# nipponjo/tts-arabic-pytorch

Measured on AMD Instinct MI355X. Metric: audio samples/sec (FastPitch+HiFi-GAN, synthetic 64-phoneme inputs), higher is better.
Workload: dtype f32

## Files before the change

tts-arabic-pytorch_amd/csrc/conv_wino4.hip:

```cpp
#include <cstdlib>
#include <cstring>

#include <algorithm>
#include <vector>

#include "conv_mfma_common.hpp"
#include "bfo.hpp"

namespace ttsamd {

typedef float w4_f32x4 __attribute__((ext_vector_type(4)));
typedef float w4_f32x2 __attribute__((ext_vector_type(2)));

template <int K, int NOCT_, int NSTAGE_, int EPI_ = 0, int PT_ = 6, int LP_ = 1>
struct Wino4Geo {
    static constexpr bool PT7 = PT_ == 7;
    static_assert(PT_ == 6 || (PT7 && (K == 7 || K == 11)), "seven-point groups: k = 7 / 11");
    static constexpr int WM = 2, WN = 2;
    static constexpr int NSF = K == 1 ? 0 : (K == 3 ? 1 : (K == 7 ? 2 : (PT7 ? 3 : 4)));
    static constexpr int NL = (!PT7 && (K == 7 || K == 1)) ? 1 : 0;
    static constexpr int GSF = PT7 ? 7 : 6;
    static constexpr int SSF = PT7 ? 4 : 3;
    static constexpr int NG = PT7 ? (K == 7 ? 13 : 20) : (K == 1 ? 4 : (K == 3 ? 6 : (K == 7 ? 16 : 23)));
    static constexpr int NGQ = PT7 ? NG : ((NG + 1) & ~1);
    static constexpr bool WSHARE = K == 1;
    static constexpr int NGW = WSHARE ? 1 : NGQ;
    static constexpr int NPL = PT7 ? (EPI_ == 3 ? 9 : 7) : ((NL || EPI_ == 3) ? 8 : 6);
    static constexpr int NPOS = K == 1 ? 4 : (K == 3 ? 6 : (K == 7 ? 10 : 14));
    static constexpr int NOCT = NOCT_, NSTAGE = NSTAGE_;
    static constexpr int NPH = PT7 ? ((K == 11 && LP_ == 2) ? 2 : 1) : (K == 11 ? 2 : 1);
    static constexpr int PH0 = PT7 ? 8 : 12;
    static constexpr int NGPM = NPH == 1 ? NG : 12;
    static_assert(NPH == 1 || (PH0 <= NGPM && NG - PH0 <= NGPM), "phase sizes");
    static constexpr int CO_BLK = WM * 32;
    static constexpr int NTUP = WN * 32;
    static constexpr int NT_BLK = 4 * NTUP;
    static constexpr int BUF4 = NOCT * 2 * NGPM * NTUP;
    static constexpr int PF = 4;
    static constexpr int NM = 4;
    __host__ __device__ static constexpr int glo(int ph) { return NPH == 1 ? 0 : PH0 * ph; }
    __host__ __device__ static constexpr int ngp(int ph) { return NPH == 1 ? NG : (ph == 0 ? PH0 : NG - PH0); }
    __host__ __device__ static constexpr int ngq(int ph) { return NPH == 1 ? NGQ : (PT7 ? ngp(ph) : 12); }
    __host__ __device__ static constexpr int gfirst(int g) {
        return g < GSF * NSF ? SSF * (g / GSF) : 3 * NSF + (g - 6 * NSF);
    }
    __host__ __device__ static constexpr int glast(int g) {
        if (PT7) return 4 * (g / 7) + (g % 7 == 6 ? 6 : 5);
        return g < 6 * NSF ? (3 * (g / 6) + 5 < NPOS ? 3 * (g / 6) + 5 : NPOS - 1) : 3 * NSF + (g - 6 * NSF);
    }
    __host__ __device__ static constexpr int plane(int g) {
        if (PT7) return g % 7;
        return g < 6 * NSF ? g % 6 : ((g - 6 * NSF) == 0 ? 0 : ((g - 6 * NSF) == 1 ? 6 : ((g - 6 * NSF) == 2 ? 7 : 5)));
    }
    __host__ __device__ static constexpr int rplane(int j) { return PT7 ? (j == 0 ? 0 : (j == 1 ? 7 : (j == 2 ? 8 : 6))) : (j == 0 ? 0 : (j == 1 ? 6 : (j == 2 ? 7 : 5))); }
    __host__ __device__ static constexpr int mlo(int ph) { return gfirst(glo(ph)); }
    __host__ __device__ static constexpr int mhi(int ph) {
        int m = 0;
        for (int g = glo(ph); g < glo(ph) + ngp(ph); ++g) m = glast(g) > m ? glast(g) : m;
        return m;
    }
    static_assert(mhi(NPH - 1) == NPOS - 1 && mlo(0) == 0, "the groups cover the window and nothing past it");
    __host__ __device__ static constexpr int npos(int ph) { return mhi(ph) - mlo(ph) + 1; }
    static constexpr int NPOSP = npos(0) > npos(NPH - 1) ? npos(0) : npos(NPH - 1);
    __host__ __device__ static constexpr int ngap(int ph) { return NOCT * ngp(ph) * NM; }
    __host__ __device__ static constexpr int sph(int ph) { return ((ph - (NSTAGE - 1)) % NPH + NPH) % NPH; }
    __host__ __device__ static constexpr int sgap(int ph) { return ngap(sph(ph)); }
    static constexpr int JSF = 10;
    __host__ __device__ static constexpr int sflo(int ph) { return glo(ph) / 7; }
    __host__ __device__ static constexpr bool inph(int ph, int g) { return g >= glo(ph) && g < glo(ph) + ngp(ph); }
    __host__ __device__ static constexpr int glast_ph(int ph) { return glo(ph) + ngp(ph) - 1; }
    __host__ __device__ static constexpr int nwj(int ph) {
        return PT7 ? JSF * (glast_ph(ph) / 7 - sflo(ph)) + (glast_ph(ph) % 7 == 0 ? 3 : JSF) : NOCT * ngp(ph);
    }
    static_assert(!PT7 || (NOCT == 1 && glo(0) % 7 <= 1 && glo(NPH - 1) % 7 <= 1 &&
                           (glast_ph(0) % 7 == 0 || glast_ph(0) % 7 >= 5) && glast_ph(NPH - 1) % 7 >= 5),
                  "seven-point phases: start on V0 / V1 of a sub-filter (the partial sums are formed per phase), end on V0 or the last row");
    __host__ __device__ static constexpr int fdiv4(int e) { return e >= 0 ? e / 4 : -((3 - e) / 4); }
    __host__ __device__ static constexpr int vlo(int ph) { return fdiv4(mlo(ph) - (K - 1) / 2); }
    __host__ __device__ static constexpr int nvec(int ph) { return fdiv4(mhi(ph) - (K - 1) / 2) - vlo(ph) + 1; }
    static constexpr int NVP = nvec(0) > nvec(NPH - 1) ? nvec(0) : nvec(NPH - 1);
    __host__ __device__ static constexpr int nljv(int ph) { return NOCT * 2 * nvec(ph); }
    static constexpr int DAV = (K == 3 || K == 1) ? 8 : 16;
    __host__ __device__ static constexpr int tw0v(int ph) { return DAV + 2 * nljv(ph); }
    __host__ __device__ static constexpr int wsv(int ph) { return (sgap(ph) - tw0v(ph)) / nwj(ph); }
    static_assert(LP_ != 1 || (wsv(0) >= 1 && wsv(NPH - 1) >= 1), "one write job per gap at most (vector loads)");
    static constexpr int RAWW = 320;
    static constexpr int NROW = 2 * NOCT;
    static constexpr int RAW_BYTES = 4 * (NROW * RAWW * 4 + 16);
    static constexpr int DAT = K == 7 ? 16 : (K == 11 ? 12 : 8);
    __host__ __device__ static constexpr int nrj(int ph) { return NROW * ((npos(ph) + 1) / 2); }
    __host__ __device__ static constexpr bool loads_in(int ph) { return ph == 0; }
    __host__ __device__ static constexpr int tr_r0(int ph) { return loads_in(ph) ? DAT + 2 * NROW : 0; }
    __host__ __device__ static constexpr int tw0t(int ph) { return tr_r0(ph) + nrj(ph) + 1; }
    __host__ __device__ static constexpr int wst(int ph) { return (sgap(ph) - tw0t(ph)) / nwj(ph); }
    static_assert(LP_ != 2 || (wst(0) >= 1 && wst(NPH - 1) >= 1), "one write job per gap at most (strip path)");
    static constexpr int QX = WSHARE ? 0 : (NOCT * ngq(0)) % PF;
    static constexpr int QMAIN = NOCT * ngq(0) - QX;
    static_assert(QX == 0 || (NPH == 1 && NOCT == 1 && QMAIN >= 2 * PF), "extra queue slots: one phase, one octet");
    static_assert((WSHARE ? NOCT : NOCT * ngq(NPH - 1)) % PF == 0 || QX != 0, "queue slots line up across steps");
    static_assert((size_t)NSTAGE * BUF4 * 16 + (LP_ == 2 ? RAW_BYTES : 0) <= 80 * 1024, "two blocks per CU");
    static_assert(NPH == 1 || NOCT == 1, "phases split an octet's groups");
};

__device__ __host__ constexpr int wino4_tile(int d, int ntup) { return (4 * ntup / (4 * d)) * (4 * d); }

template <int K, int NOCT_, int NSTAGE_, int EPI, int LP, int PT = 6>
__global__ __launch_bounds__(256, kConvMinWaves) void conv1d_wino4_f32(const ConvParams p) {
    extern __shared__ __attribute__((aligned(16))) float4 smem4[];
    using G = Wino4Geo<K, NOCT_, NSTAGE_, EPI, PT, LP>;
    constexpr bool PT7 = G::PT7;
    constexpr int WN = G::WN, NSF = G::NSF, NOCT = G::NOCT, NSTAGE = G::NSTAGE, NPL = G::NPL, NGPM = G::NGPM;
    constexpr int CO_BLK = G::CO_BLK, NTUP = G::NTUP, NT_BLK = G::NT_BLK, PF = G::PF;
    constexpr int NPH = G::NPH, NPOSP = G::NPOSP, NM = G::NM;
    constexpr bool D1 = LP == 1, TR = LP == 2;
    static_assert(D1 || TR, "window path");
    const int dil = D1 ? 1 : p.dil;
    const int nt_eff = wino4_tile(dil, NTUP), ntup_eff = nt_eff / 4;
    const int tiles_y = p.CoutP / CO_BLK;
    const int per_tile = tiles_y * p.ksplit;
    const unsigned sidx = blockIdx.x, xcd = sidx & 7u, u = sidx >> 3;
    const int yk = (int)(u % (unsigned)per_tile);
    const unsigned gt = (u / (unsigned)per_tile) * 8u + xcd;
    const int n_tiles_x = (p.Nout + nt_eff - 1) / nt_eff;
    int b = (int)(gt / (unsigned)n_tiles_x);
    int q0 = (int)(gt % (unsigned)n_tiles_x) * nt_eff;
    if (p.compact) {
        int tile = 0;
        if (!live_tile(p.lens_out, p.len_out_mul, p.Nout, nt_eff, p.batch, gt, b, tile)) return;
        b = __builtin_amdgcn_readfirstlane(b);
        q0 = __builtin_amdgcn_readfirstlane(tile) * nt_eff;
    } else if (b >= p.batch) {
        return;
    }
    const int tid = threadIdx.x, lane = tid & 63, wid = tid >> 6;
    const int wm = wid / WN, wn = wid % WN;
    const int ks = yk / tiles_y;
    const int co_blk0 = (yk - ks * tiles_y) * CO_BLK;
    int n_out = p.Nout;
    if (p.lens_out) n_out = min(n_out, (int)p.lens_out[b] * p.len_out_mul);
    if (q0 >= n_out) return;
    int in_len = p.Lin;
    if (p.lens_in) in_len = min(in_len, (int)p.lens_in[b] * p.len_in_mul);

    const int x_cs = p.x_cs, CoutP = p.CoutP;
    const int chunks_all = p.Cin / (8 * NOCT);
    const int c_beg = (int)((int64_t)ks * chunks_all / p.ksplit), n_chunks = (int)((int64_t)(ks + 1) * chunks_all / p.ksplit);
    const int n_groups = (p.Cin / 8) * G::NGW;
    const float* __restrict__ xb = p.x + (int64_t)b * p.x_bs;
    const float in_slope = p.in_slope;

    float ep_bias = 0.f;
    if (tid < CO_BLK && p.bias) ep_bias = p.bias[min(co_blk0 + tid, p.Cout - 1)];

    const int kk = lane >> 5, l31 = lane & 31;
    const int pe = wn * 32 + l31;
    const int col_e = dil == 1 ? 4 * pe : (pe / dil) * 4 * dil + pe % dil;
    f32x16 acc[NPL];
#pragma unroll
    for (int g = 0; g < NPL; ++g)
#pragma unroll
        for (int r = 0; r < 16; ++r) acc[g][r] = 0.f;
    constexpr bool preload = EPI == 3;
    if constexpr (preload) {
        const int wm_s = __builtin_amdgcn_readfirstlane(wm);
        const int row0 = co_blk0 + wm_s * 32;
        const int qv = q0 + col_e;
        const int voff = (qv < n_out ? qv : 0) * 4;
        {
            const int r_cs = p.r_cs;
            const bfo_i4 rs = bfo_rsrc(p.res + (int64_t)b * p.r_bs, (unsigned)p.Cout * (unsigned)r_cs * 4u);
            const int vk = 4 * kk * r_cs * 4;
#pragma unroll
            for (int r = 0; r < 16; ++r) {
                const w4_f32x4 t = __builtin_bit_cast(w4_f32x4, bfo_ld16(rs, voff + vk, (row0 + (r & 3) + 8 * (r >> 2)) * r_cs * 4, 0));
                acc[G::rplane(0)][r] = t.x; acc[G::rplane(1)][r] = t.y; acc[G::rplane(2)][r] = t.z; acc[G::rplane(3)][r] = t.w;
            }
        }
        if (p.mode != 0) {
            const int y_cs_ = p.y_cs;
            const bfo_i4 ys = bfo_rsrc(p.y + (int64_t)b * p.y_bs, (unsigned)p.Cout * (unsigned)y_cs_ * 4u);
            const int vk = 4 * kk * y_cs_ * 4;
#pragma unroll
            for (int r = 0; r < 16; ++r) {
                const w4_f32x4 t = __builtin_bit_cast(w4_f32x4, bfo_ld16(ys, voff + vk, (row0 + (r & 3) + 8 * (r >> 2)) * y_cs_ * 4, 0));
                acc[G::rplane(0)][r] += t.x; acc[G::rplane(1)][r] += t.y; acc[G::rplane(2)][r] += t.z; acc[G::rplane(3)][r] += t.w;
            }
        }
    }

    const bfo_i4 wrs = bfo_rsrc(K == 1 ? p.w : (PT7 ? p.w_wino44 : p.w_wino4), (unsigned)n_groups * 2u * (unsigned)CoutP * 16u);
    const int wv = (kk * CoutP + co_blk0 + wm * 32 + l31) * 16;
    const int wstep = 2 * CoutP * 16, wlast = (n_groups - 1) * wstep;
    int wso = c_beg * NOCT * G::NGW * wstep;
    w4_f32x4 aq[PF + G::QX];
    if constexpr (G::QX == 0) {
#pragma unroll
        for (int g = 0; g < PF; ++g) {
            aq[g] = __builtin_bit_cast(w4_f32x4, bfo_ld16(wrs, wv, wso, 0));
            wso = min(wso + wstep, wlast);
        }
    } else {
#pragma unroll
        for (int g = 0; g < PF + G::QX; ++g)
            aq[g] = __builtin_bit_cast(w4_f32x4, bfo_ld16(wrs, wv, min(wso + (g < PF ? g : G::QMAIN + g - PF) * wstep, wlast), 0));
    }

    const int sh = __builtin_amdgcn_readfirstlane((tid >> 7) & 1), skk = __builtin_amdgcn_readfirstlane((tid >> 6) & 1);
    w4_f32x2 sx[D1 ? 1 : NOCT][D1 ? 1 : NPOSP];
    w4_f32x4 sv[D1 ? NOCT : 1][2][D1 ? G::NVP : 1];
    w4_f32x2 ta[NOCT], tb[NOCT];
    w4_f32x2 tf[PT7 ? 5 : 1], te[PT7 ? 4 : 1], td[PT7 ? 3 : 1], th[PT7 ? 2 : 1];
    const int spe = min(lane, ntup_eff - 1);
    const int xw0 = (q0 + 4 * lane) * 4;
    constexpr int pad_c = (K - 1) / 2;
    const int ch_off = (4 * sh + skk) * x_cs;

#define TTS_VJOB_IDX(PH, J)                                                                          \
        const int nv_ = G::nvec(PH);                                                                 \
        const int ol_ = (J) / (2 * nv_), pp_ = ((J) / nv_) % 2, vi_ = (J) % nv_;
#define TTS_VLOAD_JOB(PH, J, XSO)                                                                    \
    {                                                                                                \
        TTS_VJOB_IDX(PH, J)                                                                          \
        const bfo_i4 xrs_ = bfo_rsrc(xb + ((XSO) + ch_off + (8 * ol_ + 2 * pp_) * x_cs), (unsigned)in_len * 4u);     \
        sv[ol_][pp_][vi_] = __builtin_bit_cast(w4_f32x4, bfo_ld16(xrs_, xw0 + 16 * (G::vlo(PH) + vi_), 0, 0));      \
    }
#define TTS_VACT_JOB(PH, A)                                                                          \
    {                                                                                                \
        TTS_VJOB_IDX(PH, (A) / 2)                                                                    \
        if ((A) % 2 == 0) {                                                                          \
            sv[ol_][pp_][vi_].x = bfo_lrelu(sv[ol_][pp_][vi_].x, in_slope);                          \
            sv[ol_][pp_][vi_].y = bfo_lrelu(sv[ol_][pp_][vi_].y, in_slope);                          \
        } else {                                                                                     \
            sv[ol_][pp_][vi_].z = bfo_lrelu(sv[ol_][pp_][vi_].z, in_slope);                          \
            sv[ol_][pp_][vi_].w = bfo_lrelu(sv[ol_][pp_][vi_].w, in_slope);                          \
        }                                                                                            \
    }
    float* const strip = reinterpret_cast<float*>(smem4 + NSTAGE * G::BUF4) + wid * (G::NROW * G::RAWW + 4);
    const int tr_a = (q0 - pad_c * dil) & ~3;
    const int tr_off = q0 + (dil == 1 ? 4 * spe : (spe / dil) * 4 * dil + spe % dil) - pad_c * dil - tr_a;
    w4_f32x4 rv[TR ? G::NROW : 1][2];
// ... 74 lines not shown
            const int s3 = 3 * (g_ / 6), i_ = g_ % 6;                                                \
             \
            if (i_ == 0) v2 = 4.f * TTS_SX(s3) + (TTS_SX(s3 + 4) - 5.f * TTS_SX(s3 + 2));           \
            else if (i_ == 1) {                                                                      \
                ta[ol_] = TTS_SX(s3 + 4) - 4.f * TTS_SX(s3 + 2);                                     \
                tb[ol_] = TTS_SX(s3 + 3) - 4.f * TTS_SX(s3 + 1);                                     \
                v2 = ta[ol_] + tb[ol_];                                                              \
            } else if (i_ == 2) v2 = ta[ol_] - tb[ol_];                                              \
            else if (i_ == 3) {                                                                      \
                ta[ol_] = TTS_SX(s3 + 4) - TTS_SX(s3 + 2);                                           \
                tb[ol_] = 2.f * (TTS_SX(s3 + 3) - TTS_SX(s3 + 1));                                   \
                v2 = ta[ol_] + tb[ol_];                                                              \
            } else if (i_ == 4) v2 = ta[ol_] - tb[ol_];                                              \
            else v2 = 4.f * TTS_SX(s3 + 1) + (TTS_SX(s3 + 5 < G::NPOS ? s3 + 5 : s3) - 5.f * TTS_SX(s3 + 3));           \
        } else {                                                                                     \
            v2 = TTS_SX(3 * NSF + (g_ - 6 * NSF));                                                   \
        }                                                                                            \
        if constexpr (!PT7) (WR)[2 * ((ol_ * 2 * NGPM + gl_) * NTUP)] = v2;                          \
    }

    const float4* sB = smem4 + kk * NGPM * NTUP + wn * 32 + l31;
    w4_f32x2* sW = reinterpret_cast<w4_f32x2*>(smem4 + skk * NGPM * NTUP + lane) + sh;
    float4 bq[2];

    {
#pragma unroll
        for (int st = 0; st < NSTAGE - 1; ++st) {
            const int ph = st % NPH;
            const int xso = min(c_beg + st / NPH, n_chunks - 1) * 8 * NOCT * x_cs;
            if constexpr (D1) {
#pragma unroll
                for (int J = 0; J < G::nljv(ph); ++J) TTS_VLOAD_JOB(ph, J, xso)
#pragma unroll
                for (int J = 0; J < 2 * G::nljv(ph); ++J) TTS_VACT_JOB(ph, J)
            } else {
                if (G::loads_in(ph)) {
#pragma unroll
                    for (int J = 0; J < 2 * G::NROW; ++J) TTS_TLOAD_JOB(J, xso)
#pragma unroll
                    for (int J = 0; J < 2 * G::NROW; ++J) TTS_TSTORE_JOB(J)
                }
#pragma unroll
                for (int J = 0; J < G::nrj(ph); ++J) TTS_TREAD_JOB(ph, J)
            }
            w4_f32x2* wr = sW + 2 * st * G::BUF4;
#pragma unroll
            for (int J = 0; J < G::nwj(ph); ++J) TTS_WRITE_JOB(ph, J, wr)
        }
    }
    __syncthreads();
    bq[0] = sB[0];

    int stage = 0;
    for (int c = c_beg; c < n_chunks; ++c) {
#pragma unroll
        for (int ph = 0; ph < NPH; ++ph) {
            const int tph = (ph + NSTAGE - 1) % NPH;
            const int xso = min(c + (ph + NSTAGE - 1) / NPH, n_chunks - 1) * 8 * NOCT * x_cs;
            const int stage_next = (stage + 1 == NSTAGE) ? 0 : stage + 1;
            const int stage_fill = (stage == 0) ? NSTAGE - 1 : stage - 1;
            w4_f32x2* wr = sW + 2 * stage_fill * G::BUF4;
            const float4* rd = sB + stage * G::BUF4;
            const int sn = (c + 1 < n_chunks || ph + 1 < NPH) ? stage_next : stage;
#pragma unroll
            for (int gs = 0; gs < NOCT * G::ngq(ph); ++gs) {
                const int ol = gs / G::ngq(ph), gl = gs % G::ngq(ph);
                const int qs = G::WSHARE ? ol % PF : ((G::QX && gs >= G::QMAIN) ? PF + gs - G::QMAIN : gs % PF);
                const w4_f32x4 a4 = aq[qs];
                if constexpr (G::QX != 0) {
                    const int nx = gs < G::QMAIN - PF ? gs + PF : (gs < G::QMAIN ? G::NGQ + gs + PF - G::QMAIN : G::NGQ + gs);
                    aq[qs] = __builtin_bit_cast(w4_f32x4, bfo_ld16(wrs, wv, min(wso + nx * wstep, wlast), 0));
                    if (gs == G::NGQ - 1) wso += G::NGQ * wstep;
                } else if (!G::WSHARE || gl == G::ngq(ph) - 1) {
                    aq[qs] = __builtin_bit_cast(w4_f32x4, bfo_ld16(wrs, wv, wso, 0));
                    wso = min(wso + wstep, wlast);
                }
                if (gl >= G::ngp(ph)) continue;
                const int r = ol * G::ngp(ph) + gl;
                const int cur = r & 1, nxt = cur ^ 1;
                const int plane = G::plane(G::glo(ph) + gl);
                if (r + 1 < NOCT * G::ngp(ph)) bq[nxt] = rd[(((r + 1) / G::ngp(ph)) * 2 * NGPM + (r + 1) % G::ngp(ph)) * NTUP];
                else if (NSTAGE >= 3) bq[nxt] = sB[sn * G::BUF4];
                __builtin_amdgcn_sched_barrier(0);
                const float bv[4] = {bq[cur].x, bq[cur].y, bq[cur].z, bq[cur].w};
#pragma unroll
                for (int m = 0; m < NM; ++m) {
                    acc[plane] = __builtin_amdgcn_mfma_f32_32x32x2f32(a4[m], bv[m], acc[plane], 0, 0, 0);
                    const int t = r * NM + m;
                    if constexpr (D1) {
                        if (t < G::nljv(tph)) TTS_VLOAD_JOB(tph, t, xso)
                        if (t >= G::DAV && t - G::DAV < 2 * G::nljv(tph)) TTS_VACT_JOB(tph, t - G::DAV)
                        if (t >= G::tw0v(tph) && (t - G::tw0v(tph)) % G::wsv(tph) == 0 &&
                            (t - G::tw0v(tph)) / G::wsv(tph) < G::nwj(tph))
                            TTS_WRITE_JOB(tph, (t - G::tw0v(tph)) / G::wsv(tph), wr)
                    } else {
                        if (G::loads_in(tph) && t < 2 * G::NROW) TTS_TLOAD_JOB(t, xso)
                        if (G::loads_in(tph) && t >= G::DAT && t < G::DAT + 2 * G::NROW) TTS_TSTORE_JOB(t - G::DAT)
                        if (t >= G::tr_r0(tph) && t - G::tr_r0(tph) < G::nrj(tph)) TTS_TREAD_JOB(tph, t - G::tr_r0(tph))
                        if (t >= G::tw0t(tph) && (t - G::tw0t(tph)) % G::wst(tph) == 0 && (t - G::tw0t(tph)) / G::wst(tph) < G::nwj(tph))
                            TTS_WRITE_JOB(tph, (t - G::tw0t(tph)) / G::wst(tph), wr)
                    }
                    __builtin_amdgcn_sched_barrier(0);
                }
            }
            __syncthreads();
            if (NSTAGE < 3) bq[0] = sB[sn * G::BUF4];
            else if ((NOCT * G::ngp(ph)) % 2 != 0) bq[0] = bq[1];
            stage = stage_next;
        }
    }
#undef TTS_TLOAD_JOB
#undef TTS_TSTORE_JOB
#undef TTS_TREAD_JOB
#undef TTS_VLOAD_JOB
#undef TTS_VACT_JOB
#undef TTS_VJOB_IDX
#undef TTS_SXV
#undef TTS_SX
#undef TTS_WRITE_JOB

    constexpr int LDS_F = CO_BLK * NT_BLK + CO_BLK;
    constexpr int LPR = NT_BLK / 4;
    static_assert(LPR == 64, "one wave instruction per row");
    float* ep = reinterpret_cast<float*>(smem4);
    float* epb = ep + LDS_F - CO_BLK;
    float* __restrict__ yb = p.y + (int64_t)b * p.y_bs;
    const float* __restrict__ rb = (p.res && !preload) ? p.res + (int64_t)b * p.r_bs : nullptr;
    const int mode = p.mode, relu_out = p.relu_out, Cout = p.Cout;
    const float div = p.div;
    __syncthreads();
    if (tid < CO_BLK) epb[tid] = ep_bias;
#pragma unroll
    for (int r = 0; r < 16; ++r) {
        const int row = wm * 32 + (r & 3) + 8 * (r >> 2) + 4 * kk;
        const float s12 = acc[1][r] + acc[2][r], d12 = acc[1][r] - acc[2][r];
        const float s34 = acc[3][r] + acc[4][r], d34 = acc[3][r] - acc[4][r];
        float y0 = acc[0][r] + s12 + s34;
        float y1 = d12 + 2.f * d34;
        float y2 = s12 + 4.f * s34;
        float y3 = d12 + 8.f * d34 + acc[PT7 ? 6 : 5][r];
        if constexpr (NSF == 0) { y0 = acc[0][r]; y1 = 0.f; y2 = 0.f; y3 = acc[5][r]; }
        if constexpr (PT7) {
            y0 += acc[5][r];
            y1 += 0.5f * acc[5][r];
            y2 += 0.25f * acc[5][r];
            y3 += 0.125f * acc[5][r];
            if constexpr (NPL == 9) {
                y1 += acc[7][r];
                y2 += acc[8][r];
            }
        } else if constexpr (NPL == 8) {
            y1 += acc[6][r];
            y2 += acc[7][r];
        }
        if (pe < ntup_eff) {
            if (dil == 1) {
                *reinterpret_cast<float4*>(ep + row * NT_BLK + col_e) = make_float4(y0, y1, y2, y3);
            } else {
                ep[row * NT_BLK + col_e] = y0;
                ep[row * NT_BLK + col_e + dil] = y1;
                ep[row * NT_BLK + col_e + 2 * dil] = y2;
                ep[row * NT_BLK + col_e + 3 * dil] = y3;
            }
        }
    }
    __syncthreads();
    constexpr int NR = CO_BLK / 4;
    const int col = lane * 4, q = q0 + col;
    if (q >= n_out || col >= nt_eff) return;
    const bool full = q + 3 < n_out;
    if (p.ksplit > 1) {
        float* __restrict__ pb = p.splitk_ws + ((int64_t)ks * p.batch + b) * Cout * p.Nout;
#pragma unroll 4
        for (int it = 0; it < NR; ++it) {
            const int rl = wid + it * 4;
            const int co = co_blk0 + rl;
            if (co >= Cout) continue;
            const float4 a4 = *reinterpret_cast<const float4*>(ep + rl * NT_BLK + col);
            float* yp = pb + (int64_t)co * p.Nout + q;
            if (full && (p.Nout & 3) == 0) {
                *reinterpret_cast<float4*>(yp) = a4;
            } else {
                const float v[4] = {a4.x, a4.y, a4.z, a4.w};
#pragma unroll
                for (int e = 0; e < 4; ++e)
                    if (q + e < n_out) yp[e] = v[e];
            }
        }
        return;
    }
    const float* __restrict__ scale = K == 1 ? p.scale : nullptr;
    const bool plain_act = K != 1 || (relu_out < 2 && scale == nullptr);
    if (plain_act && (preload || (!rb && mode == 0))) {
        const float lo = relu_out == 1 ? 0.f : -__builtin_inff();
        const bool do_div = preload && mode == 2;
#pragma unroll 4
        for (int it = 0; it < NR; ++it) {
            const int rl = wid + it * 4;
            const int co = co_blk0 + rl;
            if (co >= Cout) continue;
            const float bsv = epb[rl];
            const float4 a4 = *reinterpret_cast<const float4*>(ep + rl * NT_BLK + col);
            float v[4] = {fmaxf(a4.x + bsv, lo), fmaxf(a4.y + bsv, lo), fmaxf(a4.z + bsv, lo), fmaxf(a4.w + bsv, lo)};
            if (do_div) {
#pragma unroll
                for (int e = 0; e < 4; ++e) v[e] = v[e] / div;
            }
            float* yp = yb + (int64_t)co * p.y_cs + q;
            if (full) {
                *reinterpret_cast<float4*>(yp) = make_float4(v[0], v[1], v[2], v[3]);
            } else {
#pragma unroll
                for (int e = 0; e < 4; ++e)
                    if (q + e < n_out) yp[e] = v[e];
            }
        }
        return;
    }
    if constexpr (preload) return;
#pragma unroll 2
    for (int it = 0; it < NR; ++it) {
        const int rl = wid + it * 4;
        const int co = co_blk0 + rl;
        if (co >= Cout) continue;
        const float bsv = epb[rl];
        const float4 a4 = *reinterpret_cast<const float4*>(ep + rl * NT_BLK + col);
        float v[4] = {a4.x, a4.y, a4.z, a4.w};
        float* yp = yb + (int64_t)co * p.y_cs + q;
        const float* rp = rb ? rb + (int64_t)co * p.r_cs + q : nullptr;
        float rr4[4] = {0.f, 0.f, 0.f, 0.f}, pp4[4] = {0.f, 0.f, 0.f, 0.f};
        if (full) {
            if (rp) { const float4 t = *reinterpret_cast<const float4*>(rp); rr4[0] = t.x; rr4[1] = t.y; rr4[2] = t.z; rr4[3] = t.w; }
            if (mode != 0) { const float4 t = *reinterpret_cast<const float4*>(yp); pp4[0] = t.x; pp4[1] = t.y; pp4[2] = t.z; pp4[3] = t.w; }
        } else {
#pragma unroll
            for (int e = 0; e < 4; ++e)
                if (q + e < n_out) {
                    if (rp) rr4[e] = rp[e];
                    if (mode != 0) pp4[e] = yp[e];
                }
        }
        const float scv = (K == 1 && scale) ? scale[co] : 1.f;
#pragma unroll
        for (int e = 0; e < 4; ++e) {
            float x = v[e] + bsv;
            if constexpr (K == 1) {
                if (relu_out == 2) x = 0.5f * x * (1.0f + erff(x * 0.70710678118654752440f));
                x = x * scv;
            }
            x += rr4[e];
            if (relu_out == 1) x = fmaxf(x, 0.f);
            if constexpr (K == 1) { if (relu_out == 3) x = tanhf(x); }
            if (mode == 1) x = pp4[e] + x;
            else if (mode == 2) x = (pp4[e] + x) / div;
            v[e] = x;
        }
        if (full) {
            *reinterpret_cast<float4*>(yp) = make_float4(v[0], v[1], v[2], v[3]);
        } else {
#pragma unroll
            for (int e = 0; e < 4; ++e)
                if (q + e < n_out) yp[e] = v[e];
        }
    }
}

template <int K, int NOCT, int NSTAGE, int EPI, int LP, int PT = 6>
static int32_t launch_wino4_epi(const ConvParams& p, hipStream_t stream) {
    using G = Wino4Geo<K, NOCT, NSTAGE, EPI, PT, LP>;
    constexpr size_t ring = (size_t)G::NSTAGE * G::BUF4 * sizeof(float4);
    constexpr size_t epi = ((size_t)G::CO_BLK * G::NT_BLK + G::CO_BLK) * sizeof(float);
    constexpr size_t strip = LP == 2 ? (size_t)G::RAW_BYTES : 0;
    constexpr size_t lds = ring + strip > epi ? ring + strip : epi;
    static_assert(lds <= 80 * 1024, "two blocks per CU");
    static std::atomic<uint64_t> lds_done{0};
    const auto kern = conv1d_wino4_f32<K, NOCT, NSTAGE, EPI, LP, PT>;
    TTS_CHECK_HIP(lds_opt_in((const void*)kern, (int)lds, lds_done));
    const int nt = wino4_tile(p.dil, G::NTUP);
    ConvParams q = p;
    q.ksplit = EPI == 0 ? wino4_ksplit(p) : 1;
    note_conv_launch(PT == 7 ? 4 : 3, q.ksplit);
    const int64_t n_tiles = (int64_t)((p.Nout + nt - 1) / nt) * p.batch;
    const int64_t n_blocks = ((n_tiles + 7) / 8) * 8 * (p.CoutP / G::CO_BLK) * q.ksplit;
    TTS_REQUIRE(n_blocks < ((int64_t)1 << 31), "wino4: %lld blocks", (long long)n_blocks);
    dim3 grid((unsigned)n_blocks, 1, 1);
    q.compact = compact_order(p.lens_out, p.batch) ? 1 : 0;
    hipLaunchKernelGGL(kern, grid, dim3(256), lds, stream, q);
    TTS_CHECK_HIP(hipGetLastError());
    if (q.ksplit > 1) return launch_splitk_reduce(q, stream);
    return 0;
}

template <int K, int NOCT, int NSTAGE>
static int32_t launch_wino4_cfg(const ConvParams& p, hipStream_t stream) {
    if (p.dil == 1) {
        if (p.res != nullptr && wino4_ksplit(p) == 1) return launch_wino4_epi<K, NOCT, NSTAGE, 3, 1>(p, stream);
        return launch_wino4_epi<K, NOCT, NSTAGE, 0, 1>(p, stream);
    }
    return launch_wino4_epi<K, NOCT, 2, 0, 2>(p, stream);
}

template <int K>
static int32_t launch_wino44_cfg(const ConvParams& p, hipStream_t stream) {
    if (p.dil == 1) {
        if (p.res != nullptr && wino4_ksplit(p) == 1) return launch_wino4_epi<K, 1, 2, 3, 1, 7>(p, stream);
        return launch_wino4_epi<K, 1, 2, 0, 1, 7>(p, stream);
    }
    return launch_wino4_epi<K, 1, 2, 0, 2, 7>(p, stream);
}

bool wino44_wanted(const ConvParams& p) {
    if (p.w_wino44 == nullptr || (p.K != 7 && p.K != 11)) return false;
    return ((int)opt_int(OPT_WINO4, kWino4Default) & (p.K == 7 ? 32 : 64)) != 0;
}

int32_t launch_wino4(const ConvParams& p, hipStream_t stream) {
    if (wino44_wanted(p)) return p.K == 7 ? launch_wino44_cfg<7>(p, stream) : launch_wino44_cfg<11>(p, stream);
    if (p.K == 1) return launch_wino4_epi<1, 4, 2, 0, 1>(p, stream);
    if (p.K == 3) return launch_wino4_cfg<3, 2, 3>(p, stream);
    if (p.K == 7) return launch_wino4_cfg<7, 1, 2>(p, stream);
    if (p.K == 11) return launch_wino4_cfg<11, 1, 3>(p, stream);
    set_error("wino4: kernel size %d not built (1, 3, 7, 11)", p.K);
    return TTSAMD_EINVAL;
}

int wino4_block_outputs(int dil) { return wino4_tile(dil, 64); }

int wino4_ksplit(const ConvParams& p) {
    const int bo = wino4_block_outputs(p.dil);
    const int64_t blocks = (int64_t)((p.Nout + bo - 1) / bo) * (p.CoutP / 64) * p.batch;
    constexpr int sk_blocks = 192, sk_target = 224;
    if (blocks >= sk_blocks || p.splitk_ws == nullptr) return 1;
    const int n_chunks = p.Cin / (p.K == 1 ? 32 : (p.K == 3 ? 16 : 8));
    const int64_t per = (int64_t)p.batch * p.Cout * p.Nout;
    int64_t ks = std::min<int64_t>((sk_target + blocks - 1) / blocks, n_chunks / 8);
    ks = std::min<int64_t>(ks, p.splitk_floats / std::max<int64_t>(per, 1));
    return ks >= 2 ? (int)ks : 1;
}

int wino4_groups(int k) { return k == 3 ? 6 : (k == 7 ? 16 : 24); }
int wino44_groups(int k) { return k == 7 ? 13 : (k == 11 ? 20 : 0); }

void wino4_filter_groups(const float* g, int k, float* o) {
    const int nsf = k == 3 ? 1 : (k == 7 ? 2 : 4);
    for (int s = 0; s < nsf; ++s) {
        const double g0 = g[3 * s], g1 = 3 * s + 1 < k ? g[3 * s + 1] : 0.0, g2 = 3 * s + 2 < k ? g[3 * s + 2] : 0.0;
        o[6 * s] = (float)(g0 / 4);
        o[6 * s + 1] = (float)(-(g0 + g1 + g2) / 6);
        o[6 * s + 2] = (float)(-(g0 - g1 + g2) / 6);
        o[6 * s + 3] = (float)(g0 / 24 + g1 / 12 + g2 / 6);
        o[6 * s + 4] = (float)(g0 / 24 - g1 / 12 + g2 / 6);
        o[6 * s + 5] = (float)g2;
    }
    if (k == 7)
        for (int j = 0; j < 4; ++j) o[12 + j] = g[6];
}

void pack_wino4_weight(const float* w, int cout, int cin, int k, float* out) {
    const int ng = wino4_groups(k);
// ... 28 lines not shown
```

Before: 72.97 million.

## Move Winograd conv epilogue into registers and prefetch residual during last chunk

Before, the residual epilogue preloaded residual and output values into extra accumulator planes ahead of the main loop. It now peels the final chunk and issues the residual and bias loads inside the last MFMA steps, then writes outputs directly from registers. A new register-epilogue variant (EPI 4) is used for dilation-1 convs with no split-K and no residual. It skips the LDS staging round-trip and its barrier, and the LDS footprint shrinks to just the ring. The costs are extra register pressure from holding the prefetched residual (16 float4s), a larger unrolled code body, and scattered per-row global stores instead of coalesced row writes.

```diff
diff --git a/profiles/launch_classes.py b/profiles/launch_classes.py
--- /dev/null
+++ b/profiles/launch_classes.py
@@ -0,0 +1,36 @@
+import csv
+import re
+import sys
+from collections import defaultdict
+
+
+def classes(path):
+    d = defaultdict(lambda: [0, 0])
+    other = 0
+    with open(path) as f:
+        for r in csv.DictReader(f):
+            dur = int(r['End_Timestamp']) - int(r['Start_Timestamp'])
+            m = re.search(r'conv1d_wino4_f32<(\d+), (\d+), (\d+), (\d+), (\d+), (\d+)>', r['Kernel_Name'])
+            if not m:
+                other += dur
+                continue
+            k, noct, nst, epi, lp, pt = map(int, m.groups())
+            key = (pt, k, lp, 'residual' if epi == 3 else 'plain', int(r['Grid_Size_X']) // int(r['Workgroup_Size_X']))
+            d[key][0] += 1
+            d[key][1] += dur
+    return d, other
+
+
+a, oa = classes(sys.argv[1])
+b, ob = classes(sys.argv[2])
+print(f'{"groups":>6} {"k":>3} {"window":>7} {"epilogue":>9} {"blocks":>7} {"calls":>6} {"us parent":>10} {"us tree":>9} {"ratio":>6}')
+ta = tb = 0
+for key in sorted(set(a) | set(b), key=lambda t: (-t[0], t[1], t[2], t[3], t[4])):
+    ca, da = a.get(key, (0, 0))
+    cb, db = b.get(key, (0, 0))
+    ta += da
+    tb += db
+    ua, ub = (da / ca / 1e3 if ca else float('nan')), (db / cb / 1e3 if cb else float('nan'))
+    print(f'{"seven" if key[0] == 7 else "six":>6} {key[1]:3d} {"vector" if key[2] == 1 else "strip":>7} {key[3]:>9} {key[4]:7d} {max(ca, cb):6d} '
+          f'{ua:10.1f} {ub:9.1f} {ub / ua:6.3f}')
+print(f'sum over the conv1d_wino4_f32 launches: {ta / 1e6:.2f} -> {tb / 1e6:.2f} ms; every other kernel: {oa / 1e6:.2f} -> {ob / 1e6:.2f} ms (whole trace)')
diff --git a/tts-arabic-pytorch_amd/csrc/conv_wino4.hip b/tts-arabic-pytorch_amd/csrc/conv_wino4.hip
--- a/tts-arabic-pytorch_amd/csrc/conv_wino4.hip
+++ b/tts-arabic-pytorch_amd/csrc/conv_wino4.hip
@@ -12,7 +12,7 @@
 typedef float w4_f32x4 __attribute__((ext_vector_type(4)));
 typedef float w4_f32x2 __attribute__((ext_vector_type(2)));
 
-template <int K, int NOCT_, int NSTAGE_, int EPI_ = 0, int PT_ = 6, int LP_ = 1>
+template <int K, int NOCT_, int NSTAGE_, int PT_ = 6, int LP_ = 1>
 struct Wino4Geo {
     static constexpr bool PT7 = PT_ == 7;
     static_assert(PT_ == 6 || (PT7 && (K == 7 || K == 11)), "seven-point groups: k = 7 / 11");
@@ -25,7 +25,7 @@
     static constexpr int NGQ = PT7 ? NG : ((NG + 1) & ~1);
     static constexpr bool WSHARE = K == 1;
     static constexpr int NGW = WSHARE ? 1 : NGQ;
-    static constexpr int NPL = PT7 ? (EPI_ == 3 ? 9 : 7) : ((NL || EPI_ == 3) ? 8 : 6);
+    static constexpr int NPL = PT7 ? 7 : (NL ? 8 : 6);
     static constexpr int NPOS = K == 1 ? 4 : (K == 3 ? 6 : (K == 7 ? 10 : 14));
     static constexpr int NOCT = NOCT_, NSTAGE = NSTAGE_;
     static constexpr int NPH = PT7 ? ((K == 11 && LP_ == 2) ? 2 : 1) : (K == 11 ? 2 : 1);
@@ -52,7 +52,6 @@
         if (PT7) return g % 7;
         return g < 6 * NSF ? g % 6 : ((g - 6 * NSF) == 0 ? 0 : ((g - 6 * NSF) == 1 ? 6 : ((g - 6 * NSF) == 2 ? 7 : 5)));
     }
-    __host__ __device__ static constexpr int rplane(int j) { return PT7 ? (j == 0 ? 0 : (j == 1 ? 7 : (j == 2 ? 8 : 6))) : (j == 0 ? 0 : (j == 1 ? 6 : (j == 2 ? 7 : 5))); }
     __host__ __device__ static constexpr int mlo(int ph) { return gfirst(glo(ph)); }
     __host__ __device__ static constexpr int mhi(int ph) {
         int m = 0;
@@ -107,7 +106,7 @@
 template <int K, int NOCT_, int NSTAGE_, int EPI, int LP, int PT = 6>
 __global__ __launch_bounds__(256, kConvMinWaves) void conv1d_wino4_f32(const ConvParams p) {
     extern __shared__ __attribute__((aligned(16))) float4 smem4[];
-    using G = Wino4Geo<K, NOCT_, NSTAGE_, EPI, PT, LP>;
+    using G = Wino4Geo<K, NOCT_, NSTAGE_, PT, LP>;
     constexpr bool PT7 = G::PT7;
     constexpr int WN = G::WN, NSF = G::NSF, NOCT = G::NOCT, NSTAGE = G::NSTAGE, NPL = G::NPL, NGPM = G::NGPM;
     constexpr int CO_BLK = G::CO_BLK, NTUP = G::NTUP, NT_BLK = G::NT_BLK, PF = G::PF;
@@ -149,8 +148,12 @@
     const float* __restrict__ xb = p.x + (int64_t)b * p.x_bs;
     const float in_slope = p.in_slope;
 
+    constexpr bool REG = EPI >= 3, RES = EPI == 3;
+    static_assert(!REG || (LP == 1 && K != 1), "register epilogue: dilation 1, k = 3 / 7 / 11");
     float ep_bias = 0.f;
-    if (tid < CO_BLK && p.bias) ep_bias = p.bias[min(co_blk0 + tid, p.Cout - 1)];
+    if constexpr (!REG) {
+        if (tid < CO_BLK && p.bias) ep_bias = p.bias[min(co_blk0 + tid, p.Cout - 1)];
+    }
 
     const int kk = lane >> 5, l31 = lane & 31;
     const int pe = wn * 32 + l31;
@@ -160,32 +163,19 @@
     for (int g = 0; g < NPL; ++g)
 #pragma unroll
         for (int r = 0; r < 16; ++r) acc[g][r] = 0.f;
-    constexpr bool preload = EPI == 3;
-    if constexpr (preload) {
-        const int wm_s = __builtin_amdgcn_readfirstlane(wm);
-        const int row0 = co_blk0 + wm_s * 32;
-        const int qv = q0 + col_e;
-        const int voff = (qv < n_out ? qv : 0) * 4;
-        {
-            const int r_cs = p.r_cs;
-            const bfo_i4 rs = bfo_rsrc(p.res + (int64_t)b * p.r_bs, (unsigned)p.Cout * (unsigned)r_cs * 4u);
-            const int vk = 4 * kk * r_cs * 4;
-#pragma unroll
-            for (int r = 0; r < 16; ++r) {
-                const w4_f32x4 t = __builtin_bit_cast(w4_f32x4, bfo_ld16(rs, voff + vk, (row0 + (r & 3) + 8 * (r >> 2)) * r_cs * 4, 0));
-                acc[G::rplane(0)][r] = t.x; acc[G::rplane(1)][r] = t.y; acc[G::rplane(2)][r] = t.z; acc[G::rplane(3)][r] = t.w;
-            }
-        }
-        if (p.mode != 0) {
-            const int y_cs_ = p.y_cs;
-            const bfo_i4 ys = bfo_rsrc(p.y + (int64_t)b * p.y_bs, (unsigned)p.Cout * (unsigned)y_cs_ * 4u);
-            const int vk = 4 * kk * y_cs_ * 4;
-#pragma unroll
-            for (int r = 0; r < 16; ++r) {
-                const w4_f32x4 t = __builtin_bit_cast(w4_f32x4, bfo_ld16(ys, voff + vk, (row0 + (r & 3) + 8 * (r >> 2)) * y_cs_ * 4, 0));
-                acc[G::rplane(0)][r] += t.x; acc[G::rplane(1)][r] += t.y; acc[G::rplane(2)][r] += t.z; acc[G::rplane(3)][r] += t.w;
-            }
-        }
+    const int ep_row0 = REG ? co_blk0 + __builtin_amdgcn_readfirstlane(wm) * 32 : 0;
+    const int ep_voff = (q0 + col_e < n_out ? q0 + col_e : 0) * 4;
+    const int ep_rrow = ep_row0 + 4 * kk;
+    const bfo_i4 ep_rs = bfo_rsrc(RES ? p.res + (int64_t)b * p.r_bs : nullptr, RES ? (unsigned)p.Cout * (unsigned)p.r_cs * 4u : 0u);
+    const bfo_i4 ep_bs = bfo_rsrc(p.bias, (REG && p.bias) ? (unsigned)p.Cout * 4u : 0u);
+    w4_f32x4 rq[RES ? 16 : 1], bsq[REG ? 4 : 1];
+    constexpr int EP_T0 = RES ? 16 : 0;
+#define TTS_EPLOAD_JOB(T)                                                                            \
+    {                                                                                                \
+        if (RES && (T) < 16)                                                                         \
+            rq[RES ? (T) : 0] = __builtin_bit_cast(w4_f32x4, bfo_ld16(ep_rs, ep_voff + (ep_rrow + ((T) & 3) + 8 * ((T) >> 2)) * p.r_cs * 4, 0, 0)); \
+        if ((T) >= EP_T0 && (T) < EP_T0 + 4)                                                         \
+            bsq[REG ? (T) - EP_T0 : 0] = __builtin_bit_cast(w4_f32x4, bfo_ld16(ep_bs, (ep_rrow + 8 * ((T) - EP_T0)) * 4, 0, 0)); \
     }
 
     const bfo_i4 wrs = bfo_rsrc(K == 1 ? p.w : (PT7 ? p.w_wino44 : p.w_wino4), (unsigned)n_groups * 2u * (unsigned)CoutP * 16u);
@@ -366,63 +356,81 @@
     bq[0] = sB[0];
 
     int stage = 0;
-    for (int c = c_beg; c < n_chunks; ++c) {
-#pragma unroll
-        for (int ph = 0; ph < NPH; ++ph) {
-            const int tph = (ph + NSTAGE - 1) % NPH;
-            const int xso = min(c + (ph + NSTAGE - 1) / NPH, n_chunks - 1) * 8 * NOCT * x_cs;
-            const int stage_next = (stage + 1 == NSTAGE) ? 0 : stage + 1;
-            const int stage_fill = (stage == 0) ? NSTAGE - 1 : stage - 1;
-            w4_f32x2* wr = sW + 2 * stage_fill * G::BUF4;
-            const float4* rd = sB + stage * G::BUF4;
-            const int sn = (c + 1 < n_chunks || ph + 1 < NPH) ? stage_next : stage;
-#pragma unroll
-            for (int gs = 0; gs < NOCT * G::ngq(ph); ++gs) {
-                const int ol = gs / G::ngq(ph), gl = gs % G::ngq(ph);
-                const int qs = G::WSHARE ? ol % PF : ((G::QX && gs >= G::QMAIN) ? PF + gs - G::QMAIN : gs % PF);
-                const w4_f32x4 a4 = aq[qs];
-                if constexpr (G::QX != 0) {
-                    const int nx = gs < G::QMAIN - PF ? gs + PF : (gs < G::QMAIN ? G::NGQ + gs + PF - G::QMAIN : G::NGQ + gs);
-                    aq[qs] = __builtin_bit_cast(w4_f32x4, bfo_ld16(wrs, wv, min(wso + nx * wstep, wlast), 0));
-                    if (gs == G::NGQ - 1) wso += G::NGQ * wstep;
-                } else if (!G::WSHARE || gl == G::ngq(ph) - 1) {
-                    aq[qs] = __builtin_bit_cast(w4_f32x4, bfo_ld16(wrs, wv, wso, 0));
-                    wso = min(wso + wstep, wlast);
-                }
-                if (gl >= G::ngp(ph)) continue;
-                const int r = ol * G::ngp(ph) + gl;
-                const int cur = r & 1, nxt = cur ^ 1;
-                const int plane = G::plane(G::glo(ph) + gl);
-                if (r + 1 < NOCT * G::ngp(ph)) bq[nxt] = rd[(((r + 1) / G::ngp(ph)) * 2 * NGPM + (r + 1) % G::ngp(ph)) * NTUP];
-                else if (NSTAGE >= 3) bq[nxt] = sB[sn * G::BUF4];
-                __builtin_amdgcn_sched_barrier(0);
-                const float bv[4] = {bq[cur].x, bq[cur].y, bq[cur].z, bq[cur].w};
-#pragma unroll
-                for (int m = 0; m < NM; ++m) {
-                    acc[plane] = __builtin_amdgcn_mfma_f32_32x32x2f32(a4[m], bv[m], acc[plane], 0, 0, 0);
-                    const int t = r * NM + m;
-                    if constexpr (D1) {
-                        if (t < G::nljv(tph)) TTS_VLOAD_JOB(tph, t, xso)
-                        if (t >= G::DAV && t - G::DAV < 2 * G::nljv(tph)) TTS_VACT_JOB(tph, t - G::DAV)
-                        if (t >= G::tw0v(tph) && (t - G::tw0v(tph)) % G::wsv(tph) == 0 &&
-                            (t - G::tw0v(tph)) / G::wsv(tph) < G::nwj(tph))
-                            TTS_WRITE_JOB(tph, (t - G::tw0v(tph)) / G::wsv(tph), wr)
-                    } else {
-                        if (G::loads_in(tph) && t < 2 * G::NROW) TTS_TLOAD_JOB(t, xso)
-                        if (G::loads_in(tph) && t >= G::DAT && t < G::DAT + 2 * G::NROW) TTS_TSTORE_JOB(t - G::DAT)
-                        if (t >= G::tr_r0(tph) && t - G::tr_r0(tph) < G::nrj(tph)) TTS_TREAD_JOB(tph, t - G::tr_r0(tph))
-                        if (t >= G::tw0t(tph) && (t - G::tw0t(tph)) % G::wst(tph) == 0 && (t - G::tw0t(tph)) / G::wst(tph) < G::nwj(tph))
-                            TTS_WRITE_JOB(tph, (t - G::tw0t(tph)) / G::wst(tph), wr)
-                    }
-                    __builtin_amdgcn_sched_barrier(0);
-                }
-            }
-            __syncthreads();
-            if (NSTAGE < 3) bq[0] = sB[sn * G::BUF4];
-            else if ((NOCT * G::ngp(ph)) % 2 != 0) bq[0] = bq[1];
-            stage = stage_next;
-        }
-    }
+#define TTS_CHUNK_STEPS(LAST, C) \
+        _Pragma("unroll")                                                                                                                                    \
+        for (int ph = 0; ph < NPH; ++ph) {                                                                                                                   \
+            const bool peel = (LAST) && ph == NPH - 1;                                                                                                       \
+                                      \
+            const int tph = (ph + NSTAGE - 1) % NPH;                                                                                                         \
+            const int xso = min((C) + (ph + NSTAGE - 1) / NPH, n_chunks - 1) * 8 * NOCT * x_cs;                                                                \
+            const int stage_next = (stage + 1 == NSTAGE) ? 0 : stage + 1;                                                                                    \
+            const int stage_fill = (stage == 0) ? NSTAGE - 1 : stage - 1;                                                                                    \
+            w4_f32x2* wr = sW + 2 * stage_fill * G::BUF4;                                                                                                    \
+            const float4* rd = sB + stage * G::BUF4;                                                                                                         \
+            const int sn = ((C) + 1 < n_chunks || ph + 1 < NPH) ? stage_next : stage;                                                                          \
+        _Pragma("unroll")                                                                                                                                    \
+            for (int gs = 0; gs < NOCT * G::ngq(ph); ++gs) {                                                                                                 \
+                const int ol = gs / G::ngq(ph), gl = gs % G::ngq(ph);                                                                                        \
+                const int qs = G::WSHARE ? ol % PF : ((G::QX && gs >= G::QMAIN) ? PF + gs - G::QMAIN : gs % PF);                                             \
+                const w4_f32x4 a4 = aq[qs];                                                                                                                  \
+                                          \
+                if constexpr (G::QX != 0) {                                                                                                                  \
+                                            \
+                    const int nx = gs < G::QMAIN - PF ? gs + PF : (gs < G::QMAIN ? G::NGQ + gs + PF - G::QMAIN : G::NGQ + gs);                               \
+                    if (!peel || nx < G::NGQ) aq[qs] = __builtin_bit_cast(w4_f32x4, bfo_ld16(wrs, wv, min(wso + nx * wstep, wlast), 0));                     \
+                    if (gs == G::NGQ - 1) wso += G::NGQ * wstep;                                                                                             \
+                } else if ((!G::WSHARE || gl == G::ngq(ph) - 1) && (!peel || gs + PF < NOCT * G::ngq(ph))) {                                                 \
+                    aq[qs] = __builtin_bit_cast(w4_f32x4, bfo_ld16(wrs, wv, wso, 0));                                                                        \
+                    wso = min(wso + wstep, wlast);                                                                                                           \
+                }                                                                                                                                            \
+                if (gl >= G::ngp(ph)) continue;                                                     \
+                const int r = ol * G::ngp(ph) + gl;                                                                \
+                const int cur = r & 1, nxt = cur ^ 1;                                                                                                        \
+                const int plane = G::plane(G::glo(ph) + gl);                                                                                                 \
+                                                    \
+                if (r + 1 < NOCT * G::ngp(ph)) bq[nxt] = rd[(((r + 1) / G::ngp(ph)) * 2 * NGPM + (r + 1) % G::ngp(ph)) * NTUP];                              \
+                else if (NSTAGE >= 3 && !peel) bq[nxt] = sB[sn * G::BUF4];        \
+                __builtin_amdgcn_sched_barrier(0);                                                                                                           \
+                const float bv[4] = {bq[cur].x, bq[cur].y, bq[cur].z, bq[cur].w};                                                                            \
+        _Pragma("unroll")                                                                                                                                    \
+                for (int m = 0; m < NM; ++m) {                                                                                                               \
+                    acc[plane] = __builtin_amdgcn_mfma_f32_32x32x2f32(a4[m], bv[m], acc[plane], 0, 0, 0);                                                    \
+                                   \
+                                                                                             \
+                    const int t = r * NM + m;                                                                                                                \
+                    if (peel) {                                                                                                                              \
+                        TTS_EPLOAD_JOB(t)                                                                                                                    \
+                    } else if constexpr (D1) {                                                                                                               \
+                        if (t < G::nljv(tph)) TTS_VLOAD_JOB(tph, t, xso)                                                                                     \
+                        if (t >= G::DAV && t - G::DAV < 2 * G::nljv(tph)) TTS_VACT_JOB(tph, t - G::DAV)                                                      \
+                        if (t >= G::tw0v(tph) && (t - G::tw0v(tph)) % G::wsv(tph) == 0 &&                                                                    \
+                            (t - G::tw0v(tph)) / G::wsv(tph) < G::nwj(tph))                                                                                  \
+                            TTS_WRITE_JOB(tph, (t - G::tw0v(tph)) / G::wsv(tph), wr)                                                                         \
+                    } else {                                                                                                                                 \
+                        if (G::loads_in(tph) && t < 2 * G::NROW) TTS_TLOAD_JOB(t, xso)                                                                       \
+                        if (G::loads_in(tph) && t >= G::DAT && t < G::DAT + 2 * G::NROW) TTS_TSTORE_JOB(t - G::DAT)                                          \
+                        if (t >= G::tr_r0(tph) && t - G::tr_r0(tph) < G::nrj(tph)) TTS_TREAD_JOB(tph, t - G::tr_r0(tph))                                     \
+                        if (t >= G::tw0t(tph) && (t - G::tw0t(tph)) % G::wst(tph) == 0 && (t - G::tw0t(tph)) / G::wst(tph) < G::nwj(tph))                    \
+                            TTS_WRITE_JOB(tph, (t - G::tw0t(tph)) / G::wst(tph), wr)                                                                         \
+                    }                                                                                                                                        \
+                    __builtin_amdgcn_sched_barrier(0);                                                                                                       \
+                }                                                                                                                                            \
+            }                                                                                                                                                \
+            if (peel) break;                                                                                                                                 \
+            __syncthreads();                                                                                                                                 \
+            if (NSTAGE < 3) bq[0] = sB[sn * G::BUF4];                                      \
+            else if ((NOCT * G::ngp(ph)) % 2 != 0) bq[0] = bq[1];                                                                                            \
+            stage = stage_next;                                                                                                                              \
+        }
+    for (int c = c_beg; c < n_chunks - (REG ? 1 : 0); ++c) {
+        TTS_CHUNK_STEPS(false, c)
+    }
+    if constexpr (REG) {
+        const int c = n_chunks - 1;
+        TTS_CHUNK_STEPS(true, c)
+    }
+#undef TTS_CHUNK_STEPS
+#undef TTS_EPLOAD_JOB
 #undef TTS_TLOAD_JOB
 #undef TTS_TSTORE_JOB
 #undef TTS_TREAD_JOB
@@ -433,40 +441,88 @@
 #undef TTS_SX
 #undef TTS_WRITE_JOB
 
+#define TTS_OUT_QUAD(R)                                                                              \
+        const float s12 = acc[1][R] + acc[2][R], d12 = acc[1][R] - acc[2][R];                        \
+        const float s34 = acc[3][R] + acc[4][R], d34 = acc[3][R] - acc[4][R];                        \
+        float y0 = acc[0][R] + s12 + s34;                                                            \
+        float y1 = d12 + 2.f * d34;                                                                  \
+        float y2 = s12 + 4.f * s34;                                                                  \
+        float y3 = d12 + 8.f * d34 + acc[PT7 ? 6 : 5][R];                                            \
+        if constexpr (NSF == 0) { y0 = acc[0][R]; y1 = 0.f; y2 = 0.f; y3 = acc[5][R]; }               \
+        if constexpr (PT7) {                                                                   \
+            y0 += acc[5][R];                                                                         \
+            y1 += 0.5f * acc[5][R];                                                                  \
+            y2 += 0.25f * acc[5][R];                                                                 \
+            y3 += 0.125f * acc[5][R];                                                                \
+        } else if constexpr (NPL == 8) {                                                             \
+            y1 += acc[6][R];                                                                         \
+            y2 += acc[7][R];                                                                         \
+        }
+    float* __restrict__ yb = p.y + (int64_t)b * p.y_bs;
+    const int mode = p.mode, relu_out = p.relu_out, Cout = p.Cout;
+    const float div = p.div;
+    if constexpr (REG) {
+        const int q = q0 + col_e, y_cs = p.y_cs;
+        if (q >= n_out) return;
+        const bool full = q + 3 < n_out;
+        const bfo_i4 ys = bfo_rsrc(yb, (unsigned)Cout * (unsigned)y_cs * 4u);
+        const float lo = relu_out == 1 ? 0.f : -__builtin_inff();
+        constexpr int PB = NPL >= 8 ? 4 : 8;
+#pragma unroll
+        for (int h = 0; h < 16 / PB; ++h) {
+            w4_f32x4 pq[PB];
+#pragma unroll
+            for (int i = 0; i < PB; ++i) {
+                const int r = PB * h + i;
+                pq[i] = w4_f32x4{0.f, 0.f, 0.f, 0.f};
+                if (mode != 0)
+                    pq[i] = __builtin_bit_cast(w4_f32x4, bfo_ld16(ys, ep_voff + (ep_rrow + (r & 3) + 8 * (r >> 2)) * y_cs * 4, 0, 0));
+            }
+#pragma unroll
+            for (int i = 0; i < PB; ++i) {
+                const int r = PB * h + i;
+                const int co = ep_rrow + (r & 3) + 8 * (r >> 2);
+                TTS_OUT_QUAD(r)
+                w4_f32x4 v = {y0, y1, y2, y3};
+                const float bsv = bsq[REG ? r >> 2 : 0][r & 3];
+#pragma unroll
+                for (int e = 0; e < 4; ++e) {
+                    float x = v[e] + bsv;
+                    if constexpr (RES) x += rq[RES ? r : 0][e];
+                    v[e] = fmaxf(x, lo);
+                }
+                if (mode != 0) {
+                    v = pq[i] + v;
+                    if (mode == 2) {
+#pragma unroll
+                        for (int e = 0; e < 4; ++e) v[e] = v[e] / div;
+                    }
+                }
+                if (co >= Cout) continue;
+                float* yp = yb + (int64_t)co * y_cs + q;
+                if (full) {
+                    *reinterpret_cast<w4_f32x4*>(yp) = v;
+                } else {
+#pragma unroll
+                    for (int e = 0; e < 4; ++e)
+                        if (q + e < n_out) yp[e] = v[e];
+                }
+            }
+        }
+        return;
+    }
     constexpr int LDS_F = CO_BLK * NT_BLK + CO_BLK;
     constexpr int LPR = NT_BLK / 4;
     static_assert(LPR == 64, "one wave instruction per row");
     float* ep = reinterpret_cast<float*>(smem4);
     float* epb = ep + LDS_F - CO_BLK;
-    float* __restrict__ yb = p.y + (int64_t)b * p.y_bs;
-    const float* __restrict__ rb = (p.res && !preload) ? p.res + (int64_t)b * p.r_bs : nullptr;
-    const int mode = p.mode, relu_out = p.relu_out, Cout = p.Cout;
-    const float div = p.div;
+    const float* __restrict__ rb = p.res ? p.res + (int64_t)b * p.r_bs : nullptr;
     __syncthreads();
     if (tid < CO_BLK) epb[tid] = ep_bias;
 #pragma unroll
     for (int r = 0; r < 16; ++r) {
         const int row = wm * 32 + (r & 3) + 8 * (r >> 2) + 4 * kk;
-        const float s12 = acc[1][r] + acc[2][r], d12 = acc[1][r] - acc[2][r];
-        const float s34 = acc[3][r] + acc[4][r], d34 = acc[3][r] - acc[4][r];
-        float y0 = acc[0][r] + s12 + s34;
-        float y1 = d12 + 2.f * d34;
-        float y2 = s12 + 4.f * s34;
-        float y3 = d12 + 8.f * d34 + acc[PT7 ? 6 : 5][r];
-        if constexpr (NSF == 0) { y0 = acc[0][r]; y1 = 0.f; y2 = 0.f; y3 = acc[5][r]; }
-        if constexpr (PT7) {
-            y0 += acc[5][r];
-            y1 += 0.5f * acc[5][r];
-            y2 += 0.25f * acc[5][r];
-            y3 += 0.125f * acc[5][r];
-            if constexpr (NPL == 9) {
-                y1 += acc[7][r];
-                y2 += acc[8][r];
-            }
-        } else if constexpr (NPL == 8) {
-            y1 += acc[6][r];
-            y2 += acc[7][r];
-        }
+        TTS_OUT_QUAD(r)
         if (pe < ntup_eff) {
             if (dil == 1) {
                 *reinterpret_cast<float4*>(ep + row * NT_BLK + col_e) = make_float4(y0, y1, y2, y3);
@@ -478,6 +534,7 @@
             }
         }
     }
+#undef TTS_OUT_QUAD
     __syncthreads();
     constexpr int NR = CO_BLK / 4;
     const int col = lane * 4, q = q0 + col;
@@ -505,9 +562,8 @@
     }
     const float* __restrict__ scale = K == 1 ? p.scale : nullptr;
     const bool plain_act = K != 1 || (relu_out < 2 && scale == nullptr);
-    if (plain_act && (preload || (!rb && mode == 0))) {
+    if (plain_act && !rb && mode == 0) {
         const float lo = relu_out == 1 ? 0.f : -__builtin_inff();
-        const bool do_div = preload && mode == 2;
 #pragma unroll 4
         for (int it = 0; it < NR; ++it) {
             const int rl = wid + it * 4;
@@ -516,10 +572,6 @@
             const float bsv = epb[rl];
             const float4 a4 = *reinterpret_cast<const float4*>(ep + rl * NT_BLK + col);
             float v[4] = {fmaxf(a4.x + bsv, lo), fmaxf(a4.y + bsv, lo), fmaxf(a4.z + bsv, lo), fmaxf(a4.w + bsv, lo)};
-            if (do_div) {
-#pragma unroll
-                for (int e = 0; e < 4; ++e) v[e] = v[e] / div;
-            }
             float* yp = yb + (int64_t)co * p.y_cs + q;
             if (full) {
                 *reinterpret_cast<float4*>(yp) = make_float4(v[0], v[1], v[2], v[3]);
@@ -531,7 +583,6 @@
         }
         return;
     }
-    if constexpr (preload) return;
 #pragma unroll 2
     for (int it = 0; it < NR; ++it) {
         const int rl = wid + it * 4;
@@ -581,12 +632,13 @@
 
 template <int K, int NOCT, int NSTAGE, int EPI, int LP, int PT = 6>
 static int32_t launch_wino4_epi(const ConvParams& p, hipStream_t stream) {
-    using G = Wino4Geo<K, NOCT, NSTAGE, EPI, PT, LP>;
+    using G = Wino4Geo<K, NOCT, NSTAGE, PT, LP>;
     constexpr size_t ring = (size_t)G::NSTAGE * G::BUF4 * sizeof(float4);
     constexpr size_t epi = ((size_t)G::CO_BLK * G::NT_BLK + G::CO_BLK) * sizeof(float);
     constexpr size_t strip = LP == 2 ? (size_t)G::RAW_BYTES : 0;
-    constexpr size_t lds = ring + strip > epi ? ring + strip : epi;
+    constexpr size_t lds = (EPI >= 3 || ring + strip > epi) ? ring + strip : epi;
     static_assert(lds <= 80 * 1024, "two blocks per CU");
+    static_assert(EPI < 3 || lds == ring, "register epilogue: the ring sets the LDS size");
     static std::atomic<uint64_t> lds_done{0};
     const auto kern = conv1d_wino4_f32<K, NOCT, NSTAGE, EPI, LP, PT>;
     TTS_CHECK_HIP(lds_opt_in((const void*)kern, (int)lds, lds_done));
@@ -608,8 +660,9 @@
 template <int K, int NOCT, int NSTAGE>
 static int32_t launch_wino4_cfg(const ConvParams& p, hipStream_t stream) {
     if (p.dil == 1) {
-        if (p.res != nullptr && wino4_ksplit(p) == 1) return launch_wino4_epi<K, NOCT, NSTAGE, 3, 1>(p, stream);
-        return launch_wino4_epi<K, NOCT, NSTAGE, 0, 1>(p, stream);
+        if (wino4_ksplit(p) != 1) return launch_wino4_epi<K, NOCT, NSTAGE, 0, 1>(p, stream);
+        if (p.res != nullptr) return launch_wino4_epi<K, NOCT, NSTAGE, 3, 1>(p, stream);
+        return launch_wino4_epi<K, NOCT, NSTAGE, 4, 1>(p, stream);
     }
     return launch_wino4_epi<K, NOCT, 2, 0, 2>(p, stream);
 }
@@ -617,8 +670,9 @@
 template <int K>
 static int32_t launch_wino44_cfg(const ConvParams& p, hipStream_t stream) {
     if (p.dil == 1) {
-        if (p.res != nullptr && wino4_ksplit(p) == 1) return launch_wino4_epi<K, 1, 2, 3, 1, 7>(p, stream);
-        return launch_wino4_epi<K, 1, 2, 0, 1, 7>(p, stream);
+        if (wino4_ksplit(p) != 1) return launch_wino4_epi<K, 1, 2, 0, 1, 7>(p, stream);
+        if (p.res != nullptr) return launch_wino4_epi<K, 1, 2, 3, 1, 7>(p, stream);
+        return launch_wino4_epi<K, 1, 2, 4, 1, 7>(p, stream);
     }
     return launch_wino4_epi<K, 1, 2, 0, 2, 7>(p, stream);
 }
```

After: 74.05 million, median of 6. 1.01x the previous value.
